# rongzhao-zhang/EfficientQ

Measured on AMD Instinct MI355X. Metric: ptq_calibration_throughput, higher is better.
Workload: dtype i8xi8->i32 (exact) for the Gram systems and per-iteration loss convs of the layers with quantised input, f32/f64 elsewhere

## Files before the change

efficientq_amd/_lib.py:

```python
from __future__ import annotations

import ctypes as C
import os

import torch

_HERE = os.path.dirname(os.path.abspath(__file__))
LIB_PATH = os.path.join(_HERE, "libeffq_hip.so")

EFFQ_OK = 0
_ERR_NAMES = {1: "EFFQ_ERR_ARG", 2: "EFFQ_ERR_HIP", 3: "EFFQ_ERR_WORKSPACE", 4: "EFFQ_ERR_NO_DEVICE",
              5: "EFFQ_ERR_NOT_CONVERGED"}


class EffqError(RuntimeError):
    pass


class Geom(C.Structure):
    _fields_ = [(n, C.c_int32) for n in
                ("N", "C1", "C2", "D", "H", "W", "KD", "KH", "KW", "SD", "SH", "SW", "PD", "PH", "PW")]

    def out_dims(self):
        return ((self.D + 2 * self.PD - self.KD) // self.SD + 1,
# ... 47 lines not shown
SIGNATURES = {
    "effq_last_error": (C.c_char_p, []),
    "effq_version": (_I, []),
    "effq_device_count": (_I, [C.POINTER(C.c_int)]),
    "effq_quant_dequant_f32": (_I, [_P, _P, _F, _F, _I, _P, _P, _SZ, _P]),
    "effq_quant_dequant_f64path": (_I, [_P, _P, _D, _D, _I, _P, _P, _P, _SZ, _P]),
    "effq_reduce_ws_bytes": (_SZ, []),
    "effq_abs_sum_f64": (_I, [_P, _SZ, _P, _P, _P]),
    "effq_moments_f64": (_I, [_P, _SZ, _P, _P, _P]),
    "effq_alpha_stats_f64": (_I, [_P, _P, _D, _D, _I, _SZ, _P, _P, _P, _P]),
    "effq_fp_init": (_I, [_P, _P, _P]),
    "effq_fp_update": (_I, [_P, _D, _I, _P]),
    "effq_alpha_fixed_point": (_I, [_P, _SZ, _I, _D, _D, _D, _I, _I, _P, _P, _P]),
    "effq_fp_small_max": (_SZ, []),
    "effq_fixed_point_small": (_I, [_P, _P, _P, _SZ, _I, _D, _D, _D, _I, _P, _P]),
    "effq_fp_coop_max": (_SZ, []),
    "effq_fp_coop_set_spin_limit": (_I, [C.c_uint]),
    "effq_fixed_point_coop": (_I, [_P, _P, _P, _SZ, _I, _D, _D, _D, _I, _P, _P, _P]),
    "effq_fp_bucket_max": (_SZ, []),
    "effq_fp_bucket_ws_bytes": (_SZ, [_SZ]),
    "effq_fixed_point_bucket": (_I, [_P, _P, _P, _SZ, _I, _D, _D, _D, _I, _P, _P, _SZ, _P]),
    "effq_fp_bracket_ws_bytes": (_SZ, [_SZ]),
    "effq_fp_bracket_init": (_I, [_P, _P, _SZ, _I, _I, _P, _SZ, _P]),
    "effq_fp_bracket_run": (_I, [_P, _SZ, _I, _D, _D, _D, _I, _I, _P, _P, _P]),
    "effq_fp_bracket_stats": (_I, [_P, _SZ, _I, _D, _D, _P, _P, _P]),
    "effq_fp_bracket_update": (_I, [_SZ, _I, _D, _D, _D, _I, _P, _P, _P]),
    "effq_fp_traj_max": (_SZ, []),
    "effq_fp_traj_ws_bytes": (_SZ, [_SZ]),
    "effq_spd_inverse_prepare": (_I, [_P]),
    "effq_fp_traj_pred_bytes": (_SZ, []),
    "effq_fixed_point_traj": (_I, [_P, _P, _P, _SZ, _I, _D, _D, _D, _I, _P, _P, _P, _SZ, _P]),
    "effq_fixed_point_bucket_rec": (_I, [_P, _P, _P, _SZ, _I, _D, _D, _D, _I, _P, _P, _SZ, _P, _P]),
    "effq_fixed_point_coop_rec": (_I, [_P, _P, _P, _SZ, _I, _D, _D, _D, _I, _P, _P, _P, _P]),
    "effq_fp_check": (_I, [_P, _P, _P]),
    "effq_fp_channels_max_row": (_I, []),
    "effq_fixed_point_channels": (_I, [_P, _P, _P, _I, _I, _I, _D, _I, _P, _P, _P, _P]),
    "effq_fixed_point_channels_proj": (_I, [_P, _P, _P, _I, _I, _I, _D, _I, _P, _P, _P, _P, _F, _P, _P, _P, _I, _I, _D,
                                            _D, _P]),
    "effq_gram_packed_elems": (_SZ, [_I, _I]),
    "effq_gram_pack": (_I, [_P, _P, _I, _I, _P, _P]),
    "effq_gram_unpack": (_I, [_P, _I, _I, _P, _P, _P]),
    "effq_act_quant_backward": (_I, [_P, _P, _I, _P, _P, _P, _SZ, _P, _P]),
    "effq_att_classes_ws_bytes": (_SZ, []),
    "effq_att_classes": (_I, [_P, _LL, _P, _P, _P, C.POINTER(C.c_int32), _P, _P]),
    "effq_prof_enable": (_I, [_I]),
    "effq_prof_count": (_I, []),
    "effq_prof_read": (_I, [_I, C.POINTER(ProfRecord)]),
    "effq_admm_num_inverses": (_I, [_D, _D, _I, _I]),
    "effq_admm_run": (_I, [C.POINTER(AdmmRunArgs)]),
    "effq_admm_select_best": (_I, [_P, _I, _P, _P, _SZ, _SZ, _P, _P, _P, _P]),
    "effq_gram_ws_bytes": (_SZ, [_GP, _I]),
    "effq_gram_accum": (_I, [_P, _P, _P, _GP, _I, _P, _P, _I, _P, _SZ, _P]),
    "effq_gram_plan_query": (_I, [_GP, _I, _IP, _IP, _IP, _IP, _LLP, _IP, _IP]),
    "effq_gram_i8_supported": (_I, [_GP, _I]),
    "effq_gram_i8_ws_bytes": (_SZ, [_GP, _I]),
    "effq_gram_accum_i8": (_I, [_P, _P, _GP, _I, _P, _I, _P, _P, _P, _I, _LL, _P, _P, _I, _P, _SZ, _P]),
    "effq_gram_accum_i8_unw": (_I, [_P, _P, _GP, _I, _P, _I, _P, _P, _P, _I, _LL, _P, _P, _I, _P, _P, _P, _SZ, _P]),
    "effq_gram_i8_plan_query": (_I, [_GP, _I, _LL, _IP, _IP, _IP, _IP, _IP, _IP]),
    "effq_gram_i8_group_query": (_I, [_GP, _I, _LL, _IP, _IP, _IP, _IP]),
    "effq_gram_i8_set_group": (_I, [_I, _I]),
    "effq_upsample_trilinear": (_I, [_P, _I, _I, _I, _I, _I, _I, _I, _I, _P, _P]),
    "effq_gram_f64_supported": (_I, [_GP, _I]),
    "effq_gram_f64_ws_bytes": (_SZ, [_GP, _I]),
    "effq_gram_f64": (_I, [_P, _P, _GP, _I, _P, _P, _P, _SZ, _P]),
    "effq_gram_f64_plan_query": (_I, [_GP, _I, _IP, _IP, _IP, _IP]),
    "effq_gram_f64_pipelined": (_I, [_P, _P, _GP, _I]),
    "effq_gram_loss_ws_bytes": (_SZ, [_I]),
    "effq_gram_loss": (_I, [_P, _P, _P, _P, _P, _I, _I, _I, _P, _P, _SZ, _P]),
    "effq_packed_bytes": (_SZ, [_SZ, _I]),
    "effq_pack_levels": (_I, [_P, _SZ, _I, _P, _P]),
    "effq_unpack_levels": (_I, [_P, _SZ, _I, _P, _P]),
    "effq_ainv_ld": (_I, [_I]),
    "effq_fp_bracket_export_words": (_SZ, []),
    "effq_fp_bracket_export": (_I, [_P, _SZ, _P, _P, _SZ, _P]),
    "effq_fp_bracket_rebase": (_I, [_P, _P, _SZ, _P]),
    "effq_fp_bracket_import": (_I, [_P, _SZ, _P, _I, _SZ, _P, _P, _SZ, _P]),
    "effq_admm_uses_traj": (_I, [_SZ, _I]),
    "effq_gram_loss_i8_supported": (_I, [_I, _I, _I, _I]),
    "effq_gram_loss_i8_num_planes": (_I, [C.c_longlong]),
    "effq_gram_loss_i8_planes_bytes": (_SZ, [_I, _I, _I]),
    "effq_gram_loss_i8_prepare": (_I, [_P, _I, _I, _P, _I, _I, _P, _P, _P]),
    "effq_gram_loss_i8_ws_bytes": (_SZ, []),
    "effq_gram_loss_i8": (_I, [_P, _I, _P, _P, _P, _P, _P, _P, _P, _I, _I, _I, _I, _I, _I, _P, _P, _SZ, _P]),
    "effq_spd_inverse_ws_bytes": (_SZ, [_I]),
    "effq_spd_inverse": (_I, [_P, _I, _I, _D, _D, _P, _P, _SZ, _P]),
    "effq_spd_inverse_plan": (_I, [_I, _IP, _IP, _IP]),
    "effq_prox_plan_query": (_I, [_I, _I, _IP, _IP, _IP, _IP]),
    "effq_prox_ws_bytes": (_SZ, [_I, _I]),
    "effq_prox_solve": (_I, [_P, _P, _P, _P, _P, _P, _I, _I, _I, _D, _D, _P, _P, _P, _SZ, _P]),
    "effq_prox_solve_shifted": (_I, [_P, _P, _P, _P, _P, _P, _I, _I, _I, _D, _D, _D, _I, _P, _P, _P, _SZ, _P]),
    "effq_admm_presum": (_I, [_P, _P, _P, _SZ, _P]),
    "effq_admm_project_dual": (_I, [_P, _P, _P, _I, _P, _P, _F, _P, _SZ, _P]),
    "effq_conv_plan_query": (_I, [_GP, _I, _IP, _IP, _IP, _IP, _IP, _IP, _IP, _IP, _LLP]),
    "effq_conv_i8_plan_query": (_I, [_GP, _I, _IP, _IP, _IP, _IP]),
    "effq_conv_i8s_plan_query": (_I, [_GP, _I, _I, _IP, _IP, _IP, _IP, _IP, _IP, _IP]),
    "effq_conv_i8_supported": (_I, [_GP, _I, _I]),
    "effq_conv_i8s_supported": (_I, [_GP, _I, _I]),
    "effq_conv_i8s_ws_bytes": (_SZ, [_GP, _I, _I]),
    "conv3d_calib_step_i8s": (_I, [_P, _P, _P, _P, _GP, _P, _I, _P, _I, _I, _P, _P, _SZ, _P]),
    "effq_conv_i8_ws_bytes": (_SZ, [_GP]),
    "conv3d_calib_step_i8": (_I, [_P, _P, _P, _P, _GP, _P, _I, _P, _I, _P, _P, _SZ, _P]),
    "effq_conv_i8_out_supported": (_I, [_GP, _I, _I]),
    "conv3d_quant_forward_i8": (_I, [_P, _P, _P, _P, _P, _GP, _P, _I, _P, _I, _P, _P, _P, _SZ, _P]),
    "effq_conv_ws_bytes": (_SZ, [_GP]),
    "conv3d_quant_calib_step": (_I, [_P, _P, _P, _P, _P, _GP, _P, _I, _P, _P, _P, _SZ, _P]),
    "effq_adam_step": (_I, [_P, _P, _P, _P, _D, _D, _D, _D, _I, _SZ, _P]),
# ... 91 lines not shown
```

efficientq_amd/csrc/gram.hip:

```cpp
#include <stdlib.h>
#include "common.h"

namespace effq {

typedef float f32x16 __attribute__((ext_vector_type(16)));

constexpr int KC = 32;
constexpr int MB = 128;
constexpr int PS = MB + 4;

struct GramParams {
  const float* x;
  const float* att;
  const float* y;
  int N, C1, C2, D, H, W, OD, OH, OW;
  int KD, KH, KW, SD, SH, SW, PD, PH, PW;
  int T, RX, hb, E, NB, npairs;
  long long V;
  int nsplit;
  long long vox_per_split;
  int fold;
  int debug;
  double* slabs;
};

struct VoxInfo {
  int n, id0, ih0, iw0;
};

struct RowGroup {
  int kind;
  int kd, kh, kw, c0;
  int r0;
};

__device__ __forceinline__ float gram_fetch_row(const GramParams& p, int r, const VoxInfo& vi, unsigned v) {
  if (r < p.RX) {
    const int tap = r / p.C1, c = r - tap * p.C1;
    const int kw = tap % p.KW, t2 = tap / p.KW;
    const int kh = t2 % p.KH, kd = t2 / p.KH;
    const int id = vi.id0 + kd, ih = vi.ih0 + kh, iw = vi.iw0 + kw;
    if (id < 0 || id >= p.D || ih < 0 || ih >= p.H || iw < 0 || iw >= p.W) return 0.0f;
    return p.x[((((size_t)vi.n * p.D + id) * p.H + ih) * p.W + iw) * p.C1 + c];
  }
  if (r < p.RX + p.C2) return p.y[(size_t)v * p.C2 + (r - p.RX)];
  if (p.hb && r == p.RX + p.C2) return 1.0f;
  return 0.0f;
}

__device__ __forceinline__ float4 gram_fetch_cell(const GramParams& p, const RowGroup& g, const VoxInfo& vi,
                                                  unsigned v) {
  float4 val = make_float4(0.f, 0.f, 0.f, 0.f);
  if (vi.n < 0 || g.kind == 3) return val;
  if (g.kind == 0) {
    const int id = vi.id0 + g.kd, ih = vi.ih0 + g.kh, iw = vi.iw0 + g.kw;
    if (id >= 0 && id < p.D && ih >= 0 && ih < p.H && iw >= 0 && iw < p.W)
      val = *reinterpret_cast<const float4*>(p.x + ((((size_t)vi.n * p.D + id) * p.H + ih) * p.W + iw) * p.C1 + g.c0);
  } else if (g.kind == 1) {
    val = *reinterpret_cast<const float4*>(p.y + (size_t)v * p.C2 + g.c0);
  } else {
    val.x = gram_fetch_row(p, g.r0 + 0, vi, v);
    val.y = gram_fetch_row(p, g.r0 + 1, vi, v);
    val.z = gram_fetch_row(p, g.r0 + 2, vi, v);
    val.w = gram_fetch_row(p, g.r0 + 3, vi, v);
  }
  return val;
}

constexpr int GT = 512;

template <bool VEC>
__global__ __launch_bounds__(GT) void k_gram(GramParams p) {
  __shared__ __attribute__((aligned(16))) float panI[2][KC * PS];
  __shared__ __attribute__((aligned(16))) float panJ[2][KC * PS];
  __shared__ float att_s[2][KC];

// ... 133 lines not shown
    if (EFFQ_DBG(p) != 2) prefetch(more ? v0 + KC : v0);
    if (rows_live && col_live[0] && EFFQ_DBG(p) != 1) {
      const float* pi = panI[buf];
      const float* pj = diag ? panI[buf] : panJ[buf];
      if (col_live[1]) {
#pragma unroll
        for (int s = 0; s < KC / 2; ++s) {
          const int vv = 2 * s + lh;
          const float a = pi[vv * PS + wi * 32 + li] * att_s[buf][vv];
#pragma unroll
          for (int jt = 0; jt < 2; ++jt) {
            const float b = pj[vv * PS + (2 * wjh + jt) * 32 + li];
            acc[jt] = __builtin_amdgcn_mfma_f32_32x32x2f32(a, b, acc[jt], 0, 0, 0);
          }
        }
      } else {
#pragma unroll 4
        for (int s = 0; s < KC / 2; ++s) {
          const int vv = 2 * s + lh;
          const float a = pi[vv * PS + wi * 32 + li] * att_s[buf][vv];
          const float b = pj[vv * PS + (2 * wjh) * 32 + li];
          acc[0] = __builtin_amdgcn_mfma_f32_32x32x2f32(a, b, acc[0], 0, 0, 0);
        }
      }
      if (++since == fold) {
        since = 0;
#pragma unroll
        for (int jt = 0; jt < 2; ++jt)
#pragma unroll
          for (int r = 0; r < 16; ++r) {
            acc64[jt][r] += (double)acc[jt][r];
            acc[jt][r] = 0.0f;
          }
      }
    }
    if (more && EFFQ_DBG(p) != 3) stage(buf ^ 1);
    lds_barrier();
  }
#pragma unroll
  for (int jt = 0; jt < 2; ++jt)
#pragma unroll
    for (int r = 0; r < 16; ++r) acc64[jt][r] += (double)acc[jt][r];

  double* dst = p.slabs + ((size_t)blockIdx.y * p.npairs + blockIdx.x) * (size_t)(MB * MB);
#pragma unroll
  for (int jt = 0; jt < 2; ++jt)
#pragma unroll
    for (int r = 0; r < 16; ++r) {
      const int i = (r & 3) + 8 * (r >> 2) + 4 * lh;
      dst[(size_t)(wi * 32 + i) * MB + (2 * wjh + jt) * 32 + li] = acc64[jt][r];
    }
}

__global__ __launch_bounds__(256) void k_gram_finish(GramParams p, int n, float* __restrict__ A0,
                                                     float* __restrict__ B0, int accumulate) {
  const size_t nA = (size_t)n * n, nB = (size_t)p.C2 * n;
  const size_t stride = (size_t)gridDim.x * blockDim.x;
  for (size_t e = (size_t)blockIdx.x * blockDim.x + threadIdx.x; e < nA + nB; e += stride) {
    int ri, rj;
    float* dst;
    if (e < nA) {
      const int a = (int)(e / n), b = (int)(e % n);
      auto to_int = [&](int q) {
        if (p.hb && q == n - 1) return p.RX + p.C2;
        const int c = q / p.T, tap = q - c * p.T;
        return tap * p.C1 + c;
      };
      ri = to_int(a);
      rj = to_int(b);
      if (ri > rj) {
        const int t = ri;
        ri = rj;
        rj = t;
      }
      dst = A0 + e;
    } else {
      const size_t f = e - nA;
      const int c2 = (int)(f / n), b = (int)(f % n);
      if (p.hb && b == n - 1)
        ri = p.RX + p.C2;
      else {
        const int c = b / p.T, tap = b - c * p.T;
        ri = tap * p.C1 + c;
      }
      rj = p.RX + c2;
      if (ri > rj) {
        const int t = ri;
        ri = rj;
        rj = t;
      }
      dst = B0 + f;
    }
    const int I = ri / MB, J = rj / MB;
    const size_t pidx = (size_t)I * p.NB - (size_t)I * (I - 1) / 2 + (J - I);
    const size_t off = pidx * (size_t)(MB * MB) + (size_t)(ri - I * MB) * MB + (rj - J * MB);
    double s = 0.0;
    for (int k = 0; k < p.nsplit; ++k) s += p.slabs[(size_t)k * p.npairs * (size_t)(MB * MB) + off];
    const float val = (float)(2.0 * s);
    *dst = accumulate ? (*dst + val) : val;
  }
}

static int gram_plan(const effq_geom* g, int has_bias, GramParams* pp) {
  EFFQ_CHECK_ARG(g != nullptr);
  EFFQ_CHECK_ARG(g->N > 0 && g->C1 > 0 && g->C2 > 0 && g->D > 0 && g->H > 0 && g->W > 0);
  EFFQ_CHECK_ARG(g->KD >= 1 && g->KH >= 1 && g->KW >= 1 && g->SD >= 1 && g->SH >= 1 && g->SW >= 1);
  GramParams& p = *pp;
  memset(&p, 0, sizeof(p));
  p.N = g->N; p.C1 = g->C1; p.C2 = g->C2; p.D = g->D; p.H = g->H; p.W = g->W;
  p.KD = g->KD; p.KH = g->KH; p.KW = g->KW; p.SD = g->SD; p.SH = g->SH; p.SW = g->SW;
  p.PD = g->PD; p.PH = g->PH; p.PW = g->PW;
  p.OD = (g->D + 2 * g->PD - g->KD) / g->SD + 1;
  p.OH = (g->H + 2 * g->PH - g->KH) / g->SH + 1;
  p.OW = (g->W + 2 * g->PW - g->KW) / g->SW + 1;
  EFFQ_CHECK_ARG(p.OD > 0 && p.OH > 0 && p.OW > 0);
  p.T = p.KD * p.KH * p.KW;
  p.RX = p.T * p.C1;
  p.hb = has_bias ? 1 : 0;
  p.E = p.RX + p.hb + p.C2;
  p.NB = (p.E + MB - 1) / MB;
  p.npairs = p.NB * (p.NB + 1) / 2;
  p.V = (long long)p.N * p.OD * p.OH * p.OW;
  long long chunks = (p.V + KC - 1) / KC;
  long long want = (4096 + p.npairs - 1) / p.npairs;
  if (want < 1) want = 1;
  long long max_by_work = chunks / 8;
  if (max_by_work < 1) max_by_work = 1;
  long long max_by_mem = ((long long)1 << 30) / ((long long)p.npairs * MB * MB * 8);
  if (max_by_mem < 1) max_by_mem = 1;
  long long ns = want;
  if (ns > max_by_work) ns = max_by_work;
  if (ns > max_by_mem) ns = max_by_mem;
  if (ns > 65535) ns = 65535;
  long long cps = (chunks + ns - 1) / ns;
  ns = (chunks + cps - 1) / cps;
  p.nsplit = (int)ns;
  p.vox_per_split = cps * KC;
  p.fold = (p.V >= (1ll << 20)) ? 4 : 1;
  EFFQ_CHECK_ARG(p.V < (1ll << 31));
  return EFFQ_OK;
}

static bool gram_vec(const GramParams& p) { return (p.C1 & 3) == 0 && (p.C2 & 3) == 0; }

static unsigned gram_finish_blocks(const GramParams& p) {
  const int n = p.RX + p.hb;
  const size_t tot = (size_t)n * n + (size_t)p.C2 * n;
  const size_t nb = (tot + 255) / 256;
  return (unsigned)(nb > 8192 ? 8192 : nb);
}

}

using namespace effq;

extern "C" {

size_t effq_gram_ws_bytes(const effq_geom* g, int has_bias) {
  GramParams p;
  if (gram_plan(g, has_bias, &p) != EFFQ_OK) return 0;
  return (size_t)p.nsplit * p.npairs * (size_t)(MB * MB) * sizeof(double) + 256;
}

int effq_gram_accum(const float* x_ndhwc, const float* att, const float* y_ndhwc, const effq_geom* g, int has_bias,
                    float* A0, float* B0, int accumulate, void* ws, size_t ws_bytes, void* stream) {
  EFFQ_CHECK_ARG(x_ndhwc && y_ndhwc && A0 && B0 && ws);
  GramParams p;
  int rc = gram_plan(g, has_bias, &p);
  if (rc != EFFQ_OK) return rc;
  const size_t need = (size_t)p.nsplit * p.npairs * (size_t)(MB * MB) * sizeof(double);
  if (ws_bytes < need) {
    set_error("gram: workspace %zu < required %zu", ws_bytes, need);
    return EFFQ_ERR_WORKSPACE;
  }
  p.debug = effq_ablate_env("EFFQ_GRAM_DEBUG");
  p.x = x_ndhwc;
  p.att = att;
  p.y = y_ndhwc;
  p.slabs = reinterpret_cast<double*>(ws);
  hipStream_t st = as_stream(stream);
  if (gram_vec(p))
    hipLaunchKernelGGL(k_gram<true>, dim3((unsigned)p.npairs, (unsigned)p.nsplit), dim3(GT), 0, st, p);
  else
    hipLaunchKernelGGL(k_gram<false>, dim3((unsigned)p.npairs, (unsigned)p.nsplit), dim3(GT), 0, st, p);
  EFFQ_LAUNCH_CHECK();
  const int n = p.RX + p.hb;
  hipLaunchKernelGGL(k_gram_finish, dim3(gram_finish_blocks(p)), dim3(256), 0, st, p, n, A0, B0, accumulate);
  EFFQ_LAUNCH_CHECK();
  return EFFQ_OK;
}

int effq_gram_plan_query(const effq_geom* g, int has_bias, int* vec, int* nb, int* npairs, int* nsplit,
                         long long* vox_per_split, int* fold, int* finish_blocks) {
  EFFQ_CHECK_ARG(vec && nb && npairs && nsplit && vox_per_split && fold && finish_blocks);
  GramParams p;
  const int rc = gram_plan(g, has_bias, &p);
  if (rc != EFFQ_OK) return rc;
  *vec = gram_vec(p) ? 1 : 0;
  *nb = p.NB;
  *npairs = p.npairs;
  *nsplit = p.nsplit;
  *vox_per_split = p.vox_per_split;
  *fold = p.fold;
  *finish_blocks = (int)gram_finish_blocks(p);
  return EFFQ_OK;
}

}
```

efficientq_amd/hip_ops.py:

```python
from __future__ import annotations

import ctypes as C
import math
from typing import Optional, Tuple

import torch

from . import _lib
from ._lib import Geom, check

ADMM_TOL = 1e-5
FP_BRACKET_MIN = 1 << 18
DP_GATHER_AFTER = 4
DP_GATHER_MAX_BYTES = 128 << 20


def _ptr(t: Optional[torch.Tensor]):
    return None if t is None else C.c_void_p(t.data_ptr())


def to_ndhwc(x: torch.Tensor) -> torch.Tensor:
    return x.permute(0, 2, 3, 4, 1).contiguous()


# ... 331 lines not shown
        check(self.lib.effq_fixed_point_bucket_rec(_ptr(a), _ptr(b), _ptr(v), n, levels, lo, hi, ADMM_TOL, 100 * levels,
                                                   _ptr(state), _ptr(ws), ws.numel(), _ptr(pred), self.stream),
              "effq_fixed_point_bucket_rec")

    def fixed_point_coop_rec(self, a, b, v, levels: int, state, pred, lo: float = -1.0, hi: float = 1.0):
        check(self.lib.effq_fixed_point_coop_rec(_ptr(a), _ptr(b), _ptr(v), a.numel(), levels, lo, hi, ADMM_TOL,
                                                 100 * levels, _ptr(state), _ptr(self._red_ws), _ptr(pred), self.stream),
              "effq_fixed_point_coop_rec")

    @staticmethod
    def read_fp_pred(pred: torch.Tensor):
        i32 = pred[:16].view(torch.int32).cpu()
        f = pred[16:16 + 8 * 40].view(torch.float64).cpu()
        i64 = pred[16 + 8 * 40:16 + 8 * 45].view(torch.int64).cpu()
        fn = pred[16 + 8 * 45:16 + 8 * 53].view(torch.float64).cpu()
        j64 = pred[16 + 8 * 53:16 + 8 * 63].view(torch.int64).cpu()
        K = int(i32[0])
        return {"K": K, "e": int(i32[1]), "lo": f[0:8].tolist(), "hi": f[8:16].tolist(), "eps": f[16:24].tolist(),
                "eps_n": fn.tolist(), "calls": int(i64[0]), "warm_iters": int(i64[1]), "full_iters": int(i64[2]),
                "listed": int(i64[3]), "list_max": int(i64[4]), "ring_iters": int(j64[0]), "ring_listed": int(j64[1]),
                "trace_us": [(int(j64[2 + k]) - int(j64[2])) / 100.0 for k in range(5)],
                "mean_us_phase1_setup_loop": [int(j64[7 + k]) / 100.0 / max(int(i64[0]), 1) for k in range(3)]}

    def fp_check(self, state, err_flag):
        check(self.lib.effq_fp_check(_ptr(state), _ptr(err_flag), self.stream), "effq_fp_check")

    def gram(self, x_ndhwc: torch.Tensor, att: Optional[torch.Tensor], y_ndhwc: torch.Tensor, geom: Geom,
             has_bias: bool, A0: Optional[torch.Tensor] = None, B0: Optional[torch.Tensor] = None):
        x = self._f32(x_ndhwc)
        y = self._f32(y_ndhwc)
        a = self._f32(att) if att is not None else None
        _check_shapes(geom, x, y=y, att=a)
        n = geom.C1 * geom.KD * geom.KH * geom.KW + int(has_bias)
        acc = int(A0 is not None)
        if A0 is not None and (tuple(A0.shape) != (n, n) or tuple(B0.shape) != (geom.C2, n)):
            raise _lib.EffqError("gram: A0/B0 shapes do not match the geometry")
        if A0 is None:
            A0 = torch.empty(n, n, dtype=torch.float32, device=self.device)
            B0 = torch.empty(geom.C2, n, dtype=torch.float32, device=self.device)
        need = self.lib.effq_gram_ws_bytes(C.byref(geom), int(has_bias))
        ws = self._workspace("gram", need)
        check(self.lib.effq_gram_accum(_ptr(x), _ptr(a), _ptr(y), C.byref(geom), int(has_bias), _ptr(A0), _ptr(B0),
                                       acc, _ptr(ws), ws.numel(), self.stream), "effq_gram_accum")
        return A0, B0

    def gram_plan(self, geom: Geom, has_bias: bool) -> dict:
        vec, nb, npairs, nsplit, fold, fin = (C.c_int() for _ in range(6))
        vps = C.c_longlong()
        check(self.lib.effq_gram_plan_query(C.byref(geom), int(has_bias), C.byref(vec), C.byref(nb), C.byref(npairs),
                                            C.byref(nsplit), C.byref(vps), C.byref(fold), C.byref(fin)),
              "effq_gram_plan_query")
        return dict(vec=bool(vec.value), NB=nb.value, npairs=npairs.value, nsplit=nsplit.value, vox_per_split=vps.value,
                    fold=fold.value, finish_blocks=fin.value)

    def gram_i8_plan(self, geom: Geom, ncls: int = 1, n_list: int = 0) -> dict:
        out = [C.c_int() for _ in range(6)]
        check(self.lib.effq_gram_i8_plan_query(C.byref(geom), int(ncls), int(n_list), *[C.byref(o) for o in out]),
              "effq_gram_i8_plan_query")
        return dict(zip(("NB", "NBX", "npairs", "nchunks", "cps", "nsplit"), (o.value for o in out)))

    def gram_i8_groups(self, geom: Geom, ncls: int = 1, n_list: int = 0) -> dict:
        out = [C.c_int() for _ in range(4)]
        check(self.lib.effq_gram_i8_group_query(C.byref(geom), int(ncls), int(n_list), *[C.byref(o) for o in out]),
              "effq_gram_i8_group_query")
        return dict(zip(("gi", "gj", "ngroups", "grid_y"), (o.value for o in out)))

    def gram_i8_set_group(self, gi: int, gj: int) -> None:
        check(self.lib.effq_gram_i8_set_group(int(gi), int(gj)), "effq_gram_i8_set_group")

    def gram_f64_plan(self, geom: Geom, has_bias: bool) -> dict:
        out = [C.c_int() for _ in range(4)]
        check(self.lib.effq_gram_f64_plan_query(C.byref(geom), int(has_bias), *[C.byref(o) for o in out]),
              "effq_gram_f64_plan_query")
        return dict(zip(("nchunk", "grid", "ntiles", "tpw"), (o.value for o in out)))

    def gram_i8_supported(self, geom: Geom, act_levels: int) -> bool:
        return bool(self.lib.effq_gram_i8_supported(C.byref(geom), int(act_levels)))

    GRAM_I8_MAX_CLASSES = 16

    def att_classes(self, att: Optional[torch.Tensor]):
        if att is None:
            return (None, None, None, 1)
        key = (att.data_ptr(), att.numel(), att._version)
        hit = self._att_cache.get(key)
        if hit is not None:
            return hit[1]
        flat = self._f32(att).reshape(-1)
        V = flat.numel()
        lst = torch.empty(V + 128 * self.GRAM_I8_MAX_CLASSES, dtype=torch.int32, device=flat.device)
        chunk_cls = torch.empty(V // 128 + self.GRAM_I8_MAX_CLASSES, dtype=torch.int32, device=flat.device)
        cls_w = torch.empty(self.GRAM_I8_MAX_CLASSES, dtype=torch.float32, device=flat.device)
        info = (C.c_int32 * 3)()
        ws = self._workspace("att_cls", self.lib.effq_att_classes_ws_bytes())
        check(self.lib.effq_att_classes(_ptr(flat), V, _ptr(lst), _ptr(chunk_cls), _ptr(cls_w), info, _ptr(ws),
                                        self.stream), "effq_att_classes")
        k, n_list, overflow = int(info[0]), int(info[1]), int(info[2])
        res = None if overflow else (lst[:n_list], chunk_cls[: n_list // 128], cls_w[:k], k)
        if len(self._att_cache) > 16:
            self._att_cache.clear()
        self._att_cache[key] = (att, res)
        return res

    def gram_i8(self, xidx_ndhwc: torch.Tensor, att_cls, y_ndhwc: torch.Tensor, geom: Geom, has_bias: bool,
                act_alpha: torch.Tensor, act_levels: int, A0: Optional[torch.Tensor] = None,
                B0: Optional[torch.Tensor] = None, unweighted: bool = False):
# ... 1206 lines not shown
```

include/effq_hip.h:

```cpp
#ifndef EFFQ_HIP_H
#define EFFQ_HIP_H

#include <stddef.h>
#include <stdint.h>

#ifdef __cplusplus
extern "C" {
#endif

enum {
  EFFQ_OK = 0,
  EFFQ_ERR_ARG = 1,
  EFFQ_ERR_HIP = 2,
  EFFQ_ERR_WORKSPACE = 3,
  EFFQ_ERR_NO_DEVICE = 4,
  EFFQ_ERR_NOT_CONVERGED = 5
};

typedef struct effq_geom {
  int32_t N, C1, C2;
  int32_t D, H, W;
  int32_t KD, KH, KW;
  int32_t SD, SH, SW;
  int32_t PD, PH, PW;
// ... 37 lines not shown
                           double tol, int max_iter, effq_fp_state* state_dev, void* stream);
size_t effq_fp_coop_max(void);
int effq_fixed_point_coop(const float* a, const float* b, float* v_out, size_t n, int levels, double lo, double hi,
                          double tol, int max_iter, effq_fp_state* state_dev, void* ws, void* stream);
int effq_fp_coop_set_spin_limit(unsigned int polls);
size_t effq_fp_bucket_max(void);
size_t effq_fp_bucket_ws_bytes(size_t n);
int effq_fixed_point_bucket(const float* a, const float* b, float* v_out, size_t n, int levels, double lo, double hi,
                            double tol, int max_iter, effq_fp_state* state_dev, void* ws, size_t ws_bytes,
                            void* stream);

size_t effq_fp_traj_max(void);
size_t effq_fp_traj_ws_bytes(size_t n);
size_t effq_fp_traj_pred_bytes(void);
int effq_fixed_point_traj(const float* a, const float* b, float* v_out, size_t n, int levels, double lo, double hi,
                          double tol, int max_iter, effq_fp_state* state_dev, void* pred_dev, void* ws, size_t ws_bytes,
                          void* stream);
int effq_fixed_point_bucket_rec(const float* a, const float* b, float* v_out, size_t n, int levels, double lo, double hi,
                                double tol, int max_iter, effq_fp_state* state_dev, void* ws, size_t ws_bytes,
                                void* pred_dev, void* stream);
int effq_fixed_point_coop_rec(const float* a, const float* b, float* v_out, size_t n, int levels, double lo, double hi,
                              double tol, int max_iter, effq_fp_state* state_dev, void* ws, void* pred_dev, void* stream);

size_t effq_fp_bracket_ws_bytes(size_t n);
int effq_fp_bracket_init(effq_fp_state* state_dev, const double* abs_sums_dev, size_t n, int levels, int list_first,
                         void* ws, size_t ws_bytes, void* stream);
int effq_fp_bracket_run(const float* x, size_t n, int levels, double lo, double hi, double tol, int max_iter, int n_iters,
                        effq_fp_state* state_dev, void* ws, void* stream);
int effq_fp_bracket_stats(const float* x, size_t n, int levels, double lo, double hi, effq_fp_state* state_dev, void* ws,
                          void* stream);
int effq_fp_bracket_update(size_t n, int levels, double lo, double hi, double tol, int max_iter,
                           effq_fp_state* state_dev, void* ws, void* stream);
size_t effq_fp_bracket_export_words(void);
int effq_fp_bracket_export(const void* ws, size_t n, long long* out, float* list_out, size_t list_cap, void* stream);
int effq_fp_bracket_import(const void* ws_src, size_t n_src, const long long* pack_dev, int world, size_t list_cap,
                           effq_fp_state* state_dev, void* ws_dst, size_t ws_dst_bytes, void* stream);
int effq_fp_bracket_rebase(effq_fp_state* state_dev, void* ws, size_t n, void* stream);
int effq_fp_channels_max_row(void);
int effq_fixed_point_channels(const float* a, const float* b, float* v_out, int c2, int nwrow, int levels, double tol,
                              int max_iter, double* alpha_out, int32_t* iters_out, int32_t* err_flag_dev, void* stream);
int effq_fixed_point_channels_proj(const float* wstar, float* dual, float* v_out, int c2, int nwrow, int levels,
                                   double tol, int max_iter, double* alpha_out, int32_t* iters_out, int32_t* err_flag_dev,
                                   float* G, float dual_div, float* Bm, const float* B0, const float* W0, int n, int ldb,
                                   double rho_next, double eta, void* stream);

int effq_fp_check(const effq_fp_state* state_dev, int32_t* err_flag_dev, void* stream);

size_t effq_gram_ws_bytes(const effq_geom* g, int has_bias);
int effq_gram_accum(const float* x_ndhwc, const float* att, const float* y_ndhwc, const effq_geom* g,
                    int has_bias, float* A0, float* B0, int accumulate, void* ws, size_t ws_bytes,
                    void* stream);
int effq_gram_plan_query(const effq_geom* g, int has_bias, int* vec, int* nb, int* npairs, int* nsplit,
                         long long* vox_per_split, int* fold, int* finish_blocks);

int effq_gram_i8_supported(const effq_geom* g, int act_levels);
size_t effq_gram_i8_ws_bytes(const effq_geom* g, int ncls);
int effq_gram_accum_i8(const uint8_t* xidx_ndhwc, const float* y_ndhwc, const effq_geom* g, int has_bias,
                       const float* act_alpha_dev, int act_levels, const int32_t* vox_list,
                       const int32_t* chunk_cls, const float* cls_w_dev, int ncls, long long n_list,
                       float* A0, float* B0, int accumulate, void* ws, size_t ws_bytes, void* stream);
int effq_gram_accum_i8_unw(const uint8_t* xidx_ndhwc, const float* y_ndhwc, const effq_geom* g, int has_bias,
                           const float* act_alpha_dev, int act_levels, const int32_t* vox_list, const int32_t* chunk_cls,
                           const float* cls_w_dev, int ncls, long long n_list, float* A0, float* B0, int accumulate,
                           double* Au, double* Bu, void* ws, size_t ws_bytes, void* stream);
int effq_gram_i8_plan_query(const effq_geom* g, int ncls, long long n_list, int* nb, int* nbx, int* npairs, int* nchunks,
                            int* cps, int* nsplit);
int effq_gram_i8_group_query(const effq_geom* g, int ncls, long long n_list, int* gi, int* gj, int* ngroups, int* grid_y);
int effq_gram_i8_set_group(int gi, int gj);

int effq_gram_f64_supported(const effq_geom* g, int has_bias);
size_t effq_gram_f64_ws_bytes(const effq_geom* g, int has_bias);
int effq_gram_f64(const float* x_ndhwc, const float* y_ndhwc, const effq_geom* g, int has_bias, double* Au, double* Bu,
                  void* ws, size_t ws_bytes, void* stream);
int effq_gram_f64_plan_query(const effq_geom* g, int has_bias, int* nchunk, int* grid, int* ntiles, int* tpw);
int effq_gram_f64_pipelined(const float* x_ndhwc, const float* y_ndhwc, const effq_geom* g, int has_bias);

size_t effq_gram_loss_ws_bytes(int n);
int effq_gram_loss(const double* Au, const double* Bu, const double* syy_dev, const float* G, const float* b, int c2, int n,
                   int has_bias, double* sqerr_out, void* ws, size_t ws_bytes, void* stream);

int effq_gram_loss_i8_supported(int c2, int n, int has_bias, int w_levels);
int effq_gram_loss_i8_num_planes(long long kmax);
size_t effq_gram_loss_i8_planes_bytes(int n, int has_bias, int nplanes);
int effq_gram_loss_i8_prepare(const double* Au, int n, int has_bias, const float* act_alpha_dev, int act_levels,
                              int nplanes, int8_t* planes, int32_t* err_flag_dev, void* stream);
size_t effq_gram_loss_i8_ws_bytes(void);
int effq_gram_loss_i8(const int8_t* planes, int nplanes, const double* Au, const double* Bu, const double* syy_dev,
                      const int8_t* Gq, const float* b, const effq_fp_state* states, const float* act_alpha_dev,
                      int act_levels, int w_levels, int c2, int n, int has_bias, int count, double* hist_out, void* ws,
                      size_t ws_bytes, void* stream);


size_t effq_att_classes_ws_bytes(void);
int effq_att_classes(const float* att, long long V, int32_t* vox_list, int32_t* chunk_cls, float* cls_w_dev,
                     int32_t* info_host_out, void* ws, void* stream);

int effq_spd_inverse_prepare(void* stream);
int effq_ainv_ld(int n);
size_t effq_spd_inverse_ws_bytes(int n);
int effq_spd_inverse(const float* A0, int n, int has_bias, double rho, double eta, float* Ainv,
                     void* ws, size_t ws_bytes, void* stream);
int effq_spd_inverse_plan(int n, int* wide, int* nblk, int* pivot_blocks);

size_t effq_prox_ws_bytes(int c2, int n);
int effq_prox_solve(const float* B0, const float* Ainv, const float* W0, const float* b0, const float* G,
                    const float* dual, int c2, int n, int has_bias, double rho, double eta, float* wstar,
// ... 222 lines not shown
```

Measured before the change: 25.39.

## Add streamed f32 Gram kernel with incremental voxel addressing and grouped tiles

Adds a new k_gram_stream kernel for the f32 Gram accumulation. It advances voxel coordinates incrementally with precomputed carries instead of decoding each voxel index, and double-buffers float4 panel loads. When there are only two row blocks, it packs all three tile pairs into one block and deals 32x32 MFMA subtiles across the waves, with up to two subtiles per wave. The finish kernel also switches to smaller blocks and batched, unrolled slab loads so more reads are in flight across splits. The change adds code paths and alignment-dependent dispatch, and it leaves more work per block, which may raise register pressure.

Result: faster. 25.66, median of 6 (+1.1%).

```diff
diff --git a/efficientq_amd/_lib.py b/efficientq_amd/_lib.py
--- a/efficientq_amd/_lib.py
+++ b/efficientq_amd/_lib.py
@@ -123,6 +123,8 @@
     "effq_gram_ws_bytes": (_SZ, [_GP, _I]),
     "effq_gram_accum": (_I, [_P, _P, _P, _GP, _I, _P, _P, _I, _P, _SZ, _P]),
     "effq_gram_plan_query": (_I, [_GP, _I, _IP, _IP, _IP, _IP, _LLP, _IP, _IP]),
+    "effq_gram_streamed": (_I, [_P, _P, _GP, _I]),
+    "effq_gram_finish": (_I, [_GP, _I, _P, _P, _I, _P, _SZ, _P]),
     "effq_gram_i8_supported": (_I, [_GP, _I]),
     "effq_gram_i8_ws_bytes": (_SZ, [_GP, _I]),
     "effq_gram_accum_i8": (_I, [_P, _P, _GP, _I, _P, _I, _P, _P, _P, _I, _LL, _P, _P, _I, _P, _SZ, _P]),
diff --git a/efficientq_amd/csrc/gram.hip b/efficientq_amd/csrc/gram.hip
--- a/efficientq_amd/csrc/gram.hip
+++ b/efficientq_amd/csrc/gram.hip
@@ -22,6 +22,10 @@
   int fold;
   int debug;
   double* slabs;
+  int vecy;
+  int sstep[3], srad[3];
+  long long bstep, bcarry[3];
+  int group;
 };
 
 struct VoxInfo {
@@ -261,7 +265,318 @@
     }
 }
 
-__global__ __launch_bounds__(256) void k_gram_finish(GramParams p, int n, float* __restrict__ A0,
+constexpr int GS_NY = 2;
+constexpr int PANEL = KC * PS;
+
+template <bool VECY, int NS>
+__global__ __launch_bounds__(GT, NS == 1 ? 2 : 1) void k_gram_stream(GramParams p) {
+  __shared__ __attribute__((aligned(16))) float pan[2][2][PANEL];
+  __shared__ float att_s[2][KC];
+
+  const int tid = threadIdx.x, lane = tid & 63, wid = __builtin_amdgcn_readfirstlane(tid >> 6);
+  const int li = lane & 31, lh = lane >> 5;
+
+  int I = 0, J = 1;
+  if (!p.group) {
+    int rem = blockIdx.x;
+    while (rem >= p.NB - I) {
+      rem -= p.NB - I;
+      ++I;
+    }
+    J = I + rem;
+  }
+  const bool diag = (I == J);
+
+  int ns = 0, ao[2] = {0, 0}, bo[2] = {0, 0}, sp[2] = {0, 0}, sr[2] = {0, 0}, sc[2] = {0, 0};
+  {
+    const int nri = min(4, (p.E - I * MB + 31) >> 5), nrj = min(4, (p.E - J * MB + 31) >> 5);
+    int t = 0;
+    auto deal = [&](int pa, int pb, int n_a, int n_b, bool tri, int pair) {
+      for (int ri = 0; ri < n_a; ++ri)
+        for (int rj = tri ? ri : 0; rj < n_b; ++rj, ++t)
+          if ((t & 7) == wid) {
+            const int s = t >> 3;
+#pragma unroll
+            for (int q = 0; q < NS; ++q)
+              if (q == s) {
+                ao[q] = pa * PANEL + 32 * ri;
+                bo[q] = pb * PANEL + 32 * rj;
+                sp[q] = pair;
+                sr[q] = 32 * ri;
+                sc[q] = 32 * rj;
+              }
+            ++ns;
+          }
+    };
+    if (p.group) {
+      deal(0, 0, nri, nri, true, 0);
+      deal(0, 1, nri, nrj, false, 1);
+      deal(1, 1, nrj, nrj, true, 2);
+    } else {
+      deal(0, diag ? 0 : 1, nri, nrj, diag, (int)blockIdx.x);
+    }
+  }
+  ns = __builtin_amdgcn_readfirstlane(min(ns, NS));
+#pragma unroll
+  for (int q = 0; q < NS; ++q) {
+    ao[q] = __builtin_amdgcn_readfirstlane(ao[q]);
+    bo[q] = __builtin_amdgcn_readfirstlane(bo[q]);
+    sp[q] = __builtin_amdgcn_readfirstlane(sp[q]);
+    sr[q] = __builtin_amdgcn_readfirstlane(sr[q]);
+    sc[q] = __builtin_amdgcn_readfirstlane(sc[q]);
+  }
+
+  const unsigned v_begin = (unsigned)((long long)blockIdx.y * p.vox_per_split);
+  unsigned v_end = v_begin + (unsigned)p.vox_per_split;
+  if (v_end > (unsigned)p.V) v_end = (unsigned)p.V;
+  const unsigned v_last = (unsigned)p.V - 1u;
+
+  const int g = tid & 31, vsub = tid >> 5;
+  const int rload = p.RX + (VECY ? p.C2 : 0);
+  const int r0I = I * MB + 4 * g, r0J = J * MB + 4 * g;
+  const bool liveI = r0I < rload, liveJ = !diag && r0J < rload;
+  int kdI = 0, khI = 0, kwI = 0, kdJ = 0, khJ = 0, kwJ = 0;
+  long long toffI = 0, toffJ = 0;
+  const bool isxI = r0I < p.RX, isxJ = r0J < p.RX;
+  auto decode = [&](int r0, bool isx, int& kd, int& kh, int& kw, long long& toff) {
+    if (isx) {
+      const int tap = r0 / p.C1;
+      const int c0 = r0 - tap * p.C1;
+      const int t2 = tap / p.KW;
+      kw = tap - t2 * p.KW - p.PW;
+      kd = t2 / p.KH;
+      kh = t2 - kd * p.KH - p.PH;
+      kd -= p.PD;
+      toff = (((long long)kd * p.H + kh) * p.W + kw) * p.C1 + c0;
+    } else {
+      toff = r0 - p.RX;
+    }
+  };
+  if (liveI) decode(r0I, isxI, kdI, khI, kwI, toffI);
+  if (liveJ) decode(r0J, isxJ, kdJ, khJ, kwJ, toffJ);
+
+  {
+    auto constant_cell = [&](int r0) {
+      const int one = p.hb ? p.RX + p.C2 : -1;
+      return make_float4(r0 == one ? 1.f : 0.f, r0 + 1 == one ? 1.f : 0.f, r0 + 2 == one ? 1.f : 0.f,
+                         r0 + 3 == one ? 1.f : 0.f);
+    };
+#pragma unroll
+    for (int b = 0; b < 2; ++b)
+#pragma unroll
+      for (int ps = 0; ps < 2; ++ps) {
+        const int vv = vsub + 16 * ps;
+        if (!liveI) *reinterpret_cast<float4*>(&pan[b][0][vv * PS + 4 * g]) = constant_cell(r0I);
+        if (!diag && !liveJ) *reinterpret_cast<float4*>(&pan[b][1][vv * PS + 4 * g]) = constant_cell(r0J);
+      }
+  }
+
+  int yl[GS_NY], ycol[GS_NY], ydI[GS_NY], ydJ[GS_NY];
+  if (!VECY) {
+#pragma unroll
+    for (int k = 0; k < GS_NY; ++k) {
+      const int e = tid + k * GT, ec = min(e, KC * p.C2 - 1);
+      yl[k] = ec / p.C2;
+      ycol[k] = ec - yl[k] * p.C2;
+      const int r = p.RX + ycol[k], blk = r / MB;
+      const bool have = e < KC * p.C2;
+      ydI[k] = (have && blk == I) ? yl[k] * PS + (r - blk * MB) : -1;
+      ydJ[k] = (have && !diag && blk == J) ? yl[k] * PS + (r - blk * MB) : -1;
+    }
+  }
+
+  unsigned vlin[2];
+  int vd[2], vh[2], vw[2];
+  long long vbase[2], vy[2];
+#pragma unroll
+  for (int ps = 0; ps < 2; ++ps) {
+    vlin[ps] = v_begin + vsub + 16 * ps;
+    unsigned t = vlin[ps];
+    vw[ps] = (int)(t % (unsigned)p.OW) * p.SW;
+    t /= (unsigned)p.OW;
+    vh[ps] = (int)(t % (unsigned)p.OH) * p.SH;
+    t /= (unsigned)p.OH;
+    vd[ps] = (int)(t % (unsigned)p.OD) * p.SD;
+    const long long n = t / (unsigned)p.OD;
+    vbase[ps] = (((n * p.D + vd[ps]) * p.H + vh[ps]) * p.W + vw[ps]) * p.C1;
+    vy[ps] = (long long)vlin[ps] * p.C2;
+  }
+  unsigned v0p = v_begin;
+  long long yoff[GS_NY];
+  if (!VECY) {
+#pragma unroll
+    for (int k = 0; k < GS_NY; ++k) yoff[k] = (long long)(v_begin + (unsigned)yl[k]) * p.C2 + ycol[k];
+  }
+
+  float4 rI[2], rJ[2];
+  bool okI[2] = {false, false}, okJ[2] = {false, false};
+  float ry[GS_NY];
+  bool oky[GS_NY];
+  float ratt = 1.0f;
+  bool ratt_ok = false;
+#pragma unroll
+  for (int ps = 0; ps < 2; ++ps) rI[ps] = rJ[ps] = make_float4(0.f, 0.f, 0.f, 0.f);
+#pragma unroll
+  for (int k = 0; k < GS_NY; ++k) {
+    ry[k] = 0.f;
+    oky[k] = false;
+  }
+
+  auto cell_src = [&](bool isx, int kd, int kh, int kw, long long toff, int ps, bool& ok) -> const float* {
+    const int id = vd[ps] + kd, ih = vh[ps] + kh, iw = vw[ps] + kw;
+    const bool inb = id >= 0 && id < p.D && ih >= 0 && ih < p.H && iw >= 0 && iw < p.W;
+    ok = vlin[ps] < v_end && (inb || !isx);
+    const long long off = (isx ? vbase[ps] : vy[ps]) + toff;
+    return (isx ? p.x : p.y) + (ok ? off : 0ll);
+  };
+  auto prefetch = [&]() {
+    if (liveI) {
+#pragma unroll
+      for (int ps = 0; ps < 2; ++ps)
+        rI[ps] = *reinterpret_cast<const float4*>(cell_src(isxI, kdI, khI, kwI, toffI, ps, okI[ps]));
+    }
+    if (liveJ) {
+#pragma unroll
+      for (int ps = 0; ps < 2; ++ps)
+        rJ[ps] = *reinterpret_cast<const float4*>(cell_src(isxJ, kdJ, khJ, kwJ, toffJ, ps, okJ[ps]));
+    }
+    if (!VECY) {
+#pragma unroll
+      for (int k = 0; k < GS_NY; ++k) {
+        const unsigned v = v0p + (unsigned)yl[k];
+        oky[k] = v < v_end;
+        ry[k] = p.y[v <= v_last ? yoff[k] : 0ll];
+        yoff[k] += (long long)KC * p.C2;
+      }
+    }
+    {
+      const unsigned v = v0p + (unsigned)(tid & (KC - 1));
+      ratt_ok = v < v_end;
+      if (p.att != nullptr) ratt = p.att[min(v, v_last)];
+    }
+#pragma unroll
+    for (int ps = 0; ps < 2; ++ps) {
+      bool c;
+      vlin[ps] += KC;
+      vy[ps] += (long long)KC * p.C2;
+      long long b = vbase[ps] + p.bstep;
+      vw[ps] += p.sstep[2];
+      c = vw[ps] >= p.srad[2];
+      vw[ps] -= c ? p.srad[2] : 0;
+      b += c ? p.bcarry[2] : 0ll;
+      vh[ps] += p.sstep[1] + (c ? p.SH : 0);
+      c = vh[ps] >= p.srad[1];
+      vh[ps] -= c ? p.srad[1] : 0;
+      b += c ? p.bcarry[1] : 0ll;
+      vd[ps] += p.sstep[0] + (c ? p.SD : 0);
+      c = vd[ps] >= p.srad[0];
+      vd[ps] -= c ? p.srad[0] : 0;
+      b += c ? p.bcarry[0] : 0ll;
+      vbase[ps] = b;
+    }
+    v0p += KC;
+  };
+  auto keep = [](const float4& raw, bool ok) {
+    return make_float4(ok ? raw.x : 0.f, ok ? raw.y : 0.f, ok ? raw.z : 0.f, ok ? raw.w : 0.f);
+  };
+  auto stage = [&](int buf) {
+#pragma unroll
+    for (int ps = 0; ps < 2; ++ps) {
+      const int vv = vsub + 16 * ps;
+      if (liveI) *reinterpret_cast<float4*>(&pan[buf][0][vv * PS + 4 * g]) = keep(rI[ps], okI[ps]);
+      if (liveJ) *reinterpret_cast<float4*>(&pan[buf][1][vv * PS + 4 * g]) = keep(rJ[ps], okJ[ps]);
+    }
+    if (!VECY) {
+#pragma unroll
+      for (int k = 0; k < GS_NY; ++k) {
+        const float val = oky[k] ? ry[k] : 0.f;
+        if (ydI[k] >= 0) pan[buf][0][ydI[k]] = val;
+        if (ydJ[k] >= 0) pan[buf][1][ydJ[k]] = val;
+      }
+    }
+    if (tid < KC) att_s[buf][tid] = ratt_ok ? ratt : 0.0f;
+  };
+
+  double acc64[NS][16];
+  f32x16 acc[NS];
+#pragma unroll
+  for (int jt = 0; jt < NS; ++jt)
+#pragma unroll
+    for (int r = 0; r < 16; ++r) {
+      acc64[jt][r] = 0.0;
+      acc[jt][r] = 0.0f;
+    }
+  const int fold = p.fold;
+  int since = 0;
+
+  lds_barrier();
+  int buf = 0;
+  if (v_begin < v_end) {
+    prefetch();
+    stage(0);
+  }
+  lds_barrier();
+  for (unsigned v0 = v_begin; v0 < v_end; v0 += KC, buf ^= 1) {
+    const bool more = v0 + KC < v_end;
+    prefetch();
+    if (ns > 0) {
+      const float* pb = pan[buf][0];
+      bool two = false;
+      if constexpr (NS == 2) two = (ns == 2);
+      if (two) {
+        if constexpr (NS == 2) {
+#pragma unroll
+          for (int s = 0; s < KC / 2; ++s) {
+            const int vv = 2 * s + lh;
+            const float w = att_s[buf][vv];
+            const float a0 = pb[vv * PS + ao[0] + li] * w, a1 = pb[vv * PS + ao[1] + li] * w;
+            const float b0 = pb[vv * PS + bo[0] + li], b1 = pb[vv * PS + bo[1] + li];
+            acc[0] = __builtin_amdgcn_mfma_f32_32x32x2f32(a0, b0, acc[0], 0, 0, 0);
+            acc[1] = __builtin_amdgcn_mfma_f32_32x32x2f32(a1, b1, acc[1], 0, 0, 0);
+          }
+        }
+      } else {
+#pragma unroll 4
+        for (int s = 0; s < KC / 2; ++s) {
+          const int vv = 2 * s + lh;
+          const float a0 = pb[vv * PS + ao[0] + li] * att_s[buf][vv];
+          const float b0 = pb[vv * PS + bo[0] + li];
+          acc[0] = __builtin_amdgcn_mfma_f32_32x32x2f32(a0, b0, acc[0], 0, 0, 0);
+        }
+      }
+      if (++since == fold) {
+        since = 0;
+#pragma unroll
+        for (int jt = 0; jt < NS; ++jt)
+#pragma unroll
+          for (int r = 0; r < 16; ++r) {
+            acc64[jt][r] += (double)acc[jt][r];
+            acc[jt][r] = 0.0f;
+          }
+      }
+    }
+    if (more) stage(buf ^ 1);
+    lds_barrier();
+  }
+#pragma unroll
+  for (int jt = 0; jt < NS; ++jt)
+#pragma unroll
+    for (int r = 0; r < 16; ++r) acc64[jt][r] += (double)acc[jt][r];
+
+#pragma unroll
+  for (int jt = 0; jt < NS; ++jt)
+    if (jt < ns) {
+      double* dst = p.slabs + ((size_t)blockIdx.y * p.npairs + sp[jt]) * (size_t)(MB * MB);
+#pragma unroll
+      for (int r = 0; r < 16; ++r) {
+        const int i = (r & 3) + 8 * (r >> 2) + 4 * lh;
+        dst[(size_t)(sr[jt] + i) * MB + sc[jt] + li] = acc64[jt][r];
+      }
+    }
+}
+
+constexpr int GFIN_T = 64;
+__global__ __launch_bounds__(GFIN_T) void k_gram_finish(GramParams p, int n, float* __restrict__ A0,
                                                      float* __restrict__ B0, int accumulate) {
   const size_t nA = (size_t)n * n, nB = (size_t)p.C2 * n;
   const size_t stride = (size_t)gridDim.x * blockDim.x;
@@ -303,8 +618,25 @@
     const int I = ri / MB, J = rj / MB;
     const size_t pidx = (size_t)I * p.NB - (size_t)I * (I - 1) / 2 + (J - I);
     const size_t off = pidx * (size_t)(MB * MB) + (size_t)(ri - I * MB) * MB + (rj - J * MB);
+    const double* src = p.slabs + off;
+    const size_t sstride = (size_t)p.npairs * (size_t)(MB * MB);
     double s = 0.0;
-    for (int k = 0; k < p.nsplit; ++k) s += p.slabs[(size_t)k * p.npairs * (size_t)(MB * MB) + off];
+    int k = 0;
+    for (; k + 64 <= p.nsplit; k += 64) {
+      double v[64];
+#pragma unroll
+      for (int q = 0; q < 64; ++q) v[q] = src[(size_t)(k + q) * sstride];
+#pragma unroll
+      for (int q = 0; q < 64; ++q) s += v[q];
+    }
+    for (; k + 16 <= p.nsplit; k += 16) {
+      double v[16];
+#pragma unroll
+      for (int q = 0; q < 16; ++q) v[q] = src[(size_t)(k + q) * sstride];
+#pragma unroll
+      for (int q = 0; q < 16; ++q) s += v[q];
+    }
+    for (; k < p.nsplit; ++k) s += src[(size_t)k * sstride];
     const float val = (float)(2.0 * s);
     *dst = accumulate ? (*dst + val) : val;
   }
@@ -352,6 +684,12 @@
 
 static bool gram_vec(const GramParams& p) { return (p.C1 & 3) == 0 && (p.C2 & 3) == 0; }
 
+static bool gram_stream(const GramParams& p, const void* x, const void* y, int* vecy) {
+  if ((p.C1 & 3) != 0 || (reinterpret_cast<uintptr_t>(x) & 15) != 0) return false;
+  *vecy = ((p.C2 & 3) == 0 && (reinterpret_cast<uintptr_t>(y) & 15) == 0) ? 1 : 0;
+  return *vecy || KC * p.C2 <= GS_NY * GT;
+}
+
 static unsigned gram_finish_blocks(const GramParams& p) {
   const int n = p.RX + p.hb;
   const size_t tot = (size_t)n * n + (size_t)p.C2 * n;
@@ -388,13 +726,40 @@
   p.y = y_ndhwc;
   p.slabs = reinterpret_cast<double*>(ws);
   hipStream_t st = as_stream(stream);
-  if (gram_vec(p))
+  if (gram_stream(p, x_ndhwc, y_ndhwc, &p.vecy)) {
+    long long t = KC;
+    const long long sw = t % p.OW;
+    t /= p.OW;
+    const long long sh = t % p.OH;
+    t /= p.OH;
+    const long long sd = t % p.OD, sn = t / p.OD;
+    const long long fW = (long long)p.SW * p.C1, fH = (long long)p.SH * p.W * p.C1,
+                    fD = (long long)p.SD * p.H * p.W * p.C1, fN = (long long)p.D * p.H * p.W * p.C1;
+    p.sstep[0] = (int)sd * p.SD; p.sstep[1] = (int)sh * p.SH; p.sstep[2] = (int)sw * p.SW;
+    p.srad[0] = p.OD * p.SD; p.srad[1] = p.OH * p.SH; p.srad[2] = p.OW * p.SW;
+    p.bstep = sn * fN + sd * fD + sh * fH + sw * fW;
+    p.bcarry[2] = fH - p.OW * fW;
+    p.bcarry[1] = fD - p.OH * fH;
+    p.bcarry[0] = fN - p.OD * fD;
+    const int nr0 = p.NB > 1 ? 4 : (p.E + 31) / 32, nr1 = (p.E - (p.NB - 1) * MB + 31) / 32;
+    const bool one = p.NB == 1 && nr0 * (nr0 + 1) / 2 <= 8;
+    p.group = (p.NB == 2 && 10 + 4 * nr1 + nr1 * (nr1 + 1) / 2 <= 16) ? 1 : 0;
+    const dim3 grid(p.group ? 1u : (unsigned)p.npairs, (unsigned)p.nsplit);
+    if (p.vecy) {
+      if (one) hipLaunchKernelGGL((k_gram_stream<true, 1>), grid, dim3(GT), 0, st, p);
+      else hipLaunchKernelGGL((k_gram_stream<true, 2>), grid, dim3(GT), 0, st, p);
+    } else {
+      if (one) hipLaunchKernelGGL((k_gram_stream<false, 1>), grid, dim3(GT), 0, st, p);
+      else hipLaunchKernelGGL((k_gram_stream<false, 2>), grid, dim3(GT), 0, st, p);
+    }
+  } else if (gram_vec(p))
     hipLaunchKernelGGL(k_gram<true>, dim3((unsigned)p.npairs, (unsigned)p.nsplit), dim3(GT), 0, st, p);
   else
     hipLaunchKernelGGL(k_gram<false>, dim3((unsigned)p.npairs, (unsigned)p.nsplit), dim3(GT), 0, st, p);
   EFFQ_LAUNCH_CHECK();
   const int n = p.RX + p.hb;
-  hipLaunchKernelGGL(k_gram_finish, dim3(gram_finish_blocks(p)), dim3(256), 0, st, p, n, A0, B0, accumulate);
+  hipLaunchKernelGGL(k_gram_finish, dim3(gram_finish_blocks(p) * (256 / GFIN_T)), dim3(GFIN_T), 0, st, p, n, A0, B0,
+                     accumulate);
   EFFQ_LAUNCH_CHECK();
   return EFFQ_OK;
 }
@@ -415,4 +780,29 @@
   return EFFQ_OK;
 }
 
-}
+int effq_gram_finish(const effq_geom* g, int has_bias, float* A0, float* B0, int accumulate, void* ws, size_t ws_bytes,
+                     void* stream) {
+  EFFQ_CHECK_ARG(A0 && B0 && ws);
+  GramParams p;
+  int rc = gram_plan(g, has_bias, &p);
+  if (rc != EFFQ_OK) return rc;
+  const size_t need = (size_t)p.nsplit * p.npairs * (size_t)(MB * MB) * sizeof(double);
+  if (ws_bytes < need) {
+    set_error("gram: workspace %zu < required %zu", ws_bytes, need);
+    return EFFQ_ERR_WORKSPACE;
+  }
+  p.slabs = reinterpret_cast<double*>(ws);
+  const int n = p.RX + p.hb;
+  hipLaunchKernelGGL(k_gram_finish, dim3(gram_finish_blocks(p) * (256 / GFIN_T)), dim3(GFIN_T), 0, as_stream(stream), p,
+                     n, A0, B0, accumulate);
+  EFFQ_LAUNCH_CHECK();
+  return EFFQ_OK;
+}
+
+int effq_gram_streamed(const float* x_ndhwc, const float* y_ndhwc, const effq_geom* g, int has_bias) {
+  GramParams p;
+  int vecy = 0;
+  return (gram_plan(g, has_bias, &p) == EFFQ_OK && gram_stream(p, x_ndhwc, y_ndhwc, &vecy)) ? 1 : 0;
+}
+
+}
diff --git a/efficientq_amd/hip_ops.py b/efficientq_amd/hip_ops.py
--- a/efficientq_amd/hip_ops.py
+++ b/efficientq_amd/hip_ops.py
@@ -407,6 +407,9 @@
               "effq_gram_plan_query")
         return dict(vec=bool(vec.value), NB=nb.value, npairs=npairs.value, nsplit=nsplit.value, vox_per_split=vps.value,
                     fold=fold.value, finish_blocks=fin.value)
+
+    def gram_streamed(self, x_ndhwc: torch.Tensor, y_ndhwc: torch.Tensor, geom: Geom, has_bias: bool) -> bool:
+        return bool(self.lib.effq_gram_streamed(_ptr(x_ndhwc), _ptr(y_ndhwc), C.byref(geom), int(has_bias)))
 
     def gram_i8_plan(self, geom: Geom, ncls: int = 1, n_list: int = 0) -> dict:
         out = [C.c_int() for _ in range(6)]
diff --git a/include/effq_hip.h b/include/effq_hip.h
--- a/include/effq_hip.h
+++ b/include/effq_hip.h
@@ -113,6 +113,9 @@
                     void* stream);
 int effq_gram_plan_query(const effq_geom* g, int has_bias, int* vec, int* nb, int* npairs, int* nsplit,
                          long long* vox_per_split, int* fold, int* finish_blocks);
+int effq_gram_streamed(const float* x_ndhwc, const float* y_ndhwc, const effq_geom* g, int has_bias);
+int effq_gram_finish(const effq_geom* g, int has_bias, float* A0, float* B0, int accumulate, void* ws, size_t ws_bytes,
+                     void* stream);
 
 int effq_gram_i8_supported(const effq_geom* g, int act_levels);
 size_t effq_gram_i8_ws_bytes(const effq_geom* g, int ncls);
```
